# lxtGH/Video-K-Net

Hardware: AMD Instinct MI355X
Metric: frames/sec (S=3, N=100, 1024x2048) (higher is better)
Workload: dtype f32; 1 GPU; cfg2 video_knet_s3_r50: VideoKernelIterHead S=3, N=100 proposals + 17 stuff = 117 kernels, C=256, 1024x2048 frame -> 128x256 stride-8 features, ffn tracking link, x4 bilinear upsample of the final logits; streams_per_gpu=1, parallelism=frame-sharded dp1, x_storage=fp32

## Files before the change

include/vkn.h:

```cpp
#ifndef VKN_H
#define VKN_H
#include <stddef.h>
#include <stdint.h>

#ifdef __cplusplus
extern "C" {
#endif

#define VKN_VERSION 0x000600

#define VKN_OK 0
#define VKN_E_ARG (-1)
#define VKN_E_SHAPE (-2)
#define VKN_E_WORKSPACE (-3)
#define VKN_E_LAUNCH (-4)
#define VKN_E_ALIGN (-5)
#define VKN_E_RANGE (-6)

#define VKN_STATUS_RANGE 1u

#define VKN_FLAG_REF_KERNELS 1u
#define VKN_FLAG_EXACT_GEMM 2u
#define VKN_FLAG_LOGITS_HANDOFF 4u
#define VKN_FLAG_BITS_HANDOFF 16u
#define VKN_X_F32 0
#define VKN_X_F16 1
#define VKN_X_BF16 2
#define VKN_FLAG_X_F16 64u
#define VKN_FLAG_X_BF16 128u
#define VKN_FLAG_CHAIN_LAUNCHES 256u
#define VKN_FLAG_CHAIN_PERSISTENT 512u
#define VKN_FLAG_JOIN_EARLY 32768u
#define VKN_FLAG_SCALED_F16 16384u
#define VKN_FLAG_CHAIN_BF16X3 65536u
#define VKN_FLAG_CHAIN_KSPLIT 8192u
#define VKN_FLAG_SERIAL_LINK 32u
#define VKN_FLAG_CLIP_LINK 8u

#define VKN_FLAG_INIT_SEPARATE 131072u
#define VKN_FLAG_PHASE_A 1024u
#define VKN_FLAG_PHASE_B 2048u
#define VKN_FLAG_PHASE_C 4096u
#define VKN_FLAG_PHASE_MASK (VKN_FLAG_PHASE_A | VKN_FLAG_PHASE_B | VKN_FLAG_PHASE_C)

#define VKN_MAX_FCS 4

typedef struct VknDims {
// ... 366 lines not shown
```

video-k-net_amd/_lib.py:

```python
import ctypes
import os
import re
import subprocess

HERE = os.path.dirname(os.path.abspath(__file__))
CSRC = os.path.join(HERE, 'csrc')
LIBDIR = os.path.join(HERE, 'lib')
LIBPATH = os.path.join(LIBDIR, 'libvkn.so')
SOURCES = ('vkn_gather.hip', 'vkn_update.hip', 'vkn_decode.hip', 'vkn_fused.hip', 'vkn_init.hip', 'vkn_panoptic.hip', 'vkn_merge.hip', 'vkn_assign.hip', 'vkn_assign_lr.hip', 'vkn_tracker.hip', 'vkn_loss.hip', 'vkn_chain.hip', 'vkn_chain_h2.hip', 'vkn_ksplit.hip', 'vkn_train.hip', 'vkn_fpn.hip', 'vkn_optim.hip', 'vkn_tracktail.hip', 'vkn_trackloss.hip', 'vkn_gtprep.hip', 'vkn_api.hip')
HEADER = os.path.join(os.path.dirname(HERE), 'include', 'vkn.h')
TRACK_HEADER = os.path.join(os.path.dirname(HERE), 'include', 'vkn_track.h')
TRACK_TRAIN_HEADER = os.path.join(os.path.dirname(HERE), 'include', 'vkn_track_train.h')
GT_HEADER = os.path.join(os.path.dirname(HERE), 'include', 'vkn_gt.h')


class VknLibraryError(RuntimeError):
    pass


class VknError(RuntimeError):
    def __init__(self, code, msg):
        super().__init__(f'libvkn error {code}: {msg}')
        self.code = code


_SCALARS = {'int': ctypes.c_int, 'unsigned': ctypes.c_uint, 'unsigned int': ctypes.c_uint, 'size_t': ctypes.c_size_t,
            'float': ctypes.c_float, 'double': ctypes.c_double, 'long long': ctypes.c_longlong}
_POINTEES = {'void', 'char', 'unsigned char', 'int64_t'}
# ... 56 lines not shown
TRACK_PROTOS = {k: v for k, v in _protos.items() if k not in PROTOS}
TRACK_SYMBOLS = tuple(TRACK_PROTOS)
CONSTS.update({k: v for k, v in _consts.items() if k not in CONSTS})
with open(HEADER) as _f, open(TRACK_HEADER) as _g, open(TRACK_TRAIN_HEADER) as _h:
    _protos, _structs, _consts = read_header(_f.read() + '\n' + _g.read() + '\n' + _h.read())
TRACK_TRAIN_PROTOS = {k: v for k, v in _protos.items() if k not in PROTOS and k not in TRACK_PROTOS}
TRACK_TRAIN_SYMBOLS = tuple(TRACK_TRAIN_PROTOS)
TRACK_TRAIN_STRUCTS = {k: v for k, v in _structs.items() if k not in STRUCTS}
CONSTS.update({k: v for k, v in _consts.items() if k not in CONSTS})
with open(HEADER) as _f, open(TRACK_HEADER) as _g, open(TRACK_TRAIN_HEADER) as _h, open(GT_HEADER) as _i:
    _protos, _structs, _consts = read_header(_f.read() + '\n' + _g.read() + '\n' + _h.read() + '\n' + _i.read())
GT_PROTOS = {k: v for k, v in _protos.items() if k not in PROTOS and k not in TRACK_PROTOS and k not in TRACK_TRAIN_PROTOS}
GT_SYMBOLS = tuple(GT_PROTOS)
GT_STRUCTS = {k: v for k, v in _structs.items() if k not in STRUCTS and k not in TRACK_TRAIN_STRUCTS}
CONSTS.update({k: v for k, v in _consts.items() if k not in CONSTS})
GT_MAX_IMAGES = CONSTS['VKN_GT_MAX_IMAGES']
GT_MAX_CLASSES = CONSTS['VKN_GT_MAX_CLASSES']
GT_MAX_IDS = CONSTS['VKN_GT_MAX_IDS']
TRACK_LOSS_MAX_ROWS = CONSTS['VKN_TRACK_LOSS_MAX_ROWS']
TRACK_MAX_K = CONSTS['VKN_TRACK_MAX_K']
MAX_FCS = CONSTS['VKN_MAX_FCS']
SPLIT_MAX_ITEMS = CONSTS['VKN_SPLIT_MAX_ITEMS']
DW_MAX_ITEMS = CONSTS['VKN_DW_MAX_ITEMS']
ADAMW_GROUP_ROW = CONSTS['VKN_ADAMW_GROUP_ROW']
MIRRORS = {}
TRACK_TRAIN_MIRRORS = {}
GT_MIRRORS = {}


def _ctype(base, depth, where, result=False):
# ... 39 lines not shown

DEBUG_LIBPATH = os.path.join(LIBDIR, 'libvkn_debug.so')


def _hipcc(args, verbose=False, what='hipcc'):
    cmd = [os.environ.get('HIPCC', '/opt/rocm/bin/hipcc'), '--offload-arch=gfx950', *args]
    if verbose:
        print(' '.join(cmd), flush=True)
    r = subprocess.run(cmd, capture_output=True, text=True)
    if r.returncode != 0:
        raise VknLibraryError(f'{what} failed:\n' + r.stdout + r.stderr)


def _shared_deps(debug):
    exp = os.path.join(os.path.dirname(HERE), 'tools', 'experiments')
    return [HEADER, TRACK_HEADER, TRACK_TRAIN_HEADER, GT_HEADER] + ([os.path.join(exp, f) for f in os.listdir(exp)] if debug and os.path.isdir(exp) else [])


def _stale(path=None):
    path = path or LIBPATH
    if not os.path.exists(path):
        return True
    t = os.path.getmtime(path)
    deps = [os.path.join(CSRC, f) for f in os.listdir(CSRC)] + _shared_deps(path == DEBUG_LIBPATH)
    return any(os.path.getmtime(d) > t for d in deps if os.path.exists(d))


def _compile_objects(objdir, extra=(), force=False, verbose=False):
    from concurrent.futures import ThreadPoolExecutor
    os.makedirs(objdir, exist_ok=True)
    hdrs = [os.path.join(CSRC, f) for f in os.listdir(CSRC) if f.endswith('.h')] + _shared_deps('-DVKN_DEBUG' in extra)
# ... 38 lines not shown
    global _USE_DEBUG
    if _LIB is not None:
        raise VknLibraryError('use_debug() must be called before the library is first used')
    _USE_DEBUG = True


def lib():
    global _LIB
    if _LIB is not None:
        return _LIB
    path = DEBUG_LIBPATH if _USE_DEBUG else LIBPATH
    if not os.path.exists(path):
        raise VknLibraryError(f'{path} is missing — run `python -c "import __graft_entry__ as g; g.build()"` '
                              '(there is deliberately no CPU fallback)')
    L = ctypes.CDLL(path)
    for name, (result, params) in {**PROTOS, **TRACK_PROTOS, **TRACK_TRAIN_PROTOS, **GT_PROTOS}.items():
        fn = getattr(L, name)
        fn.restype = _ctype(*result, name, result=True)
        fn.argtypes = [POINTER_EXCEPTIONS.get((name, p)) or _ctype(base, depth, name) for p, base, depth in params]
    for name, mirror in {**MIRRORS, **TRACK_TRAIN_MIRRORS, **GT_MIRRORS}.items():
        probe = 'vkn_sizeof_' + re.sub(r'(?<!^)(?=[A-Z])', '_', name[3:]).lower()
        if probe not in PROTOS and probe not in TRACK_TRAIN_PROTOS and probe not in GT_PROTOS:
            raise VknLibraryError(f'include/vkn.h declares struct {name} without its size probe {probe}()')
        if getattr(L, probe)() != ctypes.sizeof(mirror):
            raise VknLibraryError(f'{path} does not match include/vkn.h: struct {name} is {getattr(L, probe)()} bytes in the library, '
                                  f'{ctypes.sizeof(mirror)} in the header')
    _LIB = L
    return L


def check(code):
# ... 3 lines not shown
```

video-k-net_amd/csrc/vkn_api.hip:

```cpp
#include "../../include/vkn.h"
#include "vkn_common.h"
#include "vkn_launch.h"

namespace {

struct Carver {
    char* base;
    size_t off;
    template <class T>
    T* take(size_t n) {
        off = (off + 255) & ~(size_t)255;
        T* p = base ? reinterpret_cast<T*>(base + off) : nullptr;
        off += n * sizeof(T);
        return p;
    }
};

inline bool aligned16(const void* p) { return (reinterpret_cast<uintptr_t>(p) & 15) == 0; }
inline int npt_of(int N) { return (N + 31) / 32 * 32; }

struct StageWs {
    float *part, *cntp, *xraw, *cnt, *xfeat, *params, *inputf, *ig, *ug, *f, *obj1, *qkv, *ao, *obj2, *h, *partial, *t1, *t2,
        *maskfeat, *kb, *kern32, *lq, *lkv, *lobj, *lupd, *lf;
    _Float16 *kfh, *kfl;
// ... 18 lines not shown
    const VknStageWeights* w = nullptr;
    const float *x = nullptr, *obj_in = nullptr;
    float *obj_out = nullptr, *cls_logits = nullptr, *x_feat_out = nullptr;
    bool cls_sigmoid = false;
    MasksFrom from = FROM_LOGITS;
    const float *masks_in = nullptr, *xfeat_in = nullptr;
    const unsigned* bits_in = nullptr;
    MasksTo to = TO_LOGITS;
    float* masks_out = nullptr;
    unsigned* bits_out = nullptr;
    float *kern_out = nullptr, *kb_out = nullptr;
    hipEvent_t prof0 = nullptr, prof1 = nullptr, obj_ready = nullptr;
    float* up_out = nullptr;
    int up_stride = 0, up_chunk = 0;
    bool* up_done = nullptr;
    const float* prev_obj = nullptr;
    float* track_out = nullptr;
    const VknStageWeights* link_pre = nullptr;
    const float* prev_pre = nullptr;
    const VknStageWeights* link_track = nullptr;
    int track_src = 0;
    bool keep_xfeat = false;
    const void* touch_next = nullptr;
    size_t touch_next_bytes = 0;
};

struct PrepW {
    const void *ft, *ftT, *dyn, *inp, *ig, *ug, *fc, *attn_in, *attn_out, *ffn1, *ffn2, *cls_fc[VKN_MAX_FCS], *fc_cls,
        *mask_fc[VKN_MAX_FCS], *fc_mask, *pa_in, *pa_in_kv, *pa_out, *lffn1, *lffn2;
    const void *dynft, *dec;
// ... 306 lines not shown
    const VknStageWeights* lw = link_track ? link_track : w;
    PrepW pw;
    VKN_TRY(carve_pw(d, lw, flags, &pw));
    return run_link(d, lw, pw, cur, prev, out, s, st, link_track ? (track_src == 2 ? cur : xfeat) : nullptr, flags);
}

int run_gather(const VknDims* d, const float* x, const float* masks, const unsigned* bits, const StageWs& s, unsigned flags,
               hipStream_t st, const void* touch = nullptr, size_t touch_bytes = 0) {
    const int B = d->B, N = d->N, C = d->C, P = d->H * d->W, xdt = xdt_of(flags);
    if (flags & VKN_FLAG_REF_KERNELS) return vkn_launch_gather_ref(x, masks, d->thr_logit, s.xraw, s.cnt, B, N, C, P, st);
    if (bits) return vkn_launch_gather_bits(x, bits, s.xraw, s.cnt, s.part, s.cntp, B, N, C, P, st, xdt, s.status, touch, touch_bytes);
    return vkn_launch_gather(x, masks, d->thr_logit, s.xraw, s.cnt, s.part, s.cntp, B, N, C, P, st, xdt, s.status, touch, touch_bytes);
}

int final_decode(const VknDims* d, const float* x, const StageWs& s, const float* kb, float* masks_out, unsigned flags,
                 hipStream_t st, hipEvent_t prof0, hipEvent_t prof1, float* up_out, int up_stride, int up_chunk, bool* up_done) {
    const int B = d->B, N = d->N, C = d->C, P = d->H * d->W;
    if ((flags & VKN_FLAG_REF_KERNELS) || (P & 1)) return vkn_launch_decode_ref(x, s.kern32, kb, masks_out, B, N, C, P, st);
    const int ch = (up_out && up_chunk > 0 && up_chunk < B) ? up_chunk : B;
    const size_t NPTC = (size_t)npt_of(N) * C;
    for (int b0 = 0; b0 < B; b0 += ch) {
        const int bn = (B - b0 < ch) ? B - b0 : ch;
        const float* xb = reinterpret_cast<const float*>(reinterpret_cast<const char*>(x) + (size_t)b0 * C * P * (xdt_of(flags) ? 2 : 4));
        if (b0 == 0 && prof0 && hipEventRecord(prof0, st) != hipSuccess) return VKN_E_LAUNCH;
        VKN_TRY(vkn_launch_decode(xb, s.kfh + b0 * NPTC, s.kfl + b0 * NPTC, kb ? kb + (size_t)b0 * N : nullptr,
                                  masks_out + (size_t)b0 * N * P, bn, N, C, P, st, xdt_of(flags)));
        if (b0 == 0 && prof1 && hipEventRecord(prof1, st) != hipSuccess) return VKN_E_LAUNCH;
        if (ch < B)
            VKN_TRY(vkn_launch_upsample(masks_out + (size_t)b0 * N * P,
                                        (flags & VKN_FLAG_SCALED_F16) ? reinterpret_cast<float*>(reinterpret_cast<_Float16*>(up_out) + (size_t)b0 * N * P * up_stride * up_stride)
                                                                      : up_out + (size_t)b0 * N * P * up_stride * up_stride,
                                        bn * N, d->H, d->W, up_stride, st, (flags & VKN_FLAG_SCALED_F16) ? 1 : 0));
    }
    if (ch < B && up_done) *up_done = true;
    return VKN_OK;
}

inline int persistent_min_row_tiles(const PrepW& pw, unsigned flags) {
    return (!(flags & VKN_FLAG_CHAIN_BF16X3) && pw.h2_scale && pw.h2[VKN_H2_DYNFT]) ? 22 : 64;
}
inline unsigned pw_off(const VknStageWeights* w, const void* p) {
    return (unsigned)(static_cast<const char*>(p) - static_cast<const char*>(w->prepared));
}
inline bool chain_weights_ok(const PrepW& pw, bool have_cls) {
    return pw.dynft && pw.dyn && pw.dec && pw.inp && pw.ig && pw.ug && pw.fc && pw.attn_in && pw.attn_out && pw.ffn1 && pw.ffn2 &&
           pw.cls_fc[0] && pw.mask_fc[0] && (!have_cls || pw.fc_cls);
}
inline bool chain_stage_ok(const VknDims* d, const VknStageWeights* w, const PrepW& pw, bool have_cls) {
    return chain_shape_ok(d) && w->prepared && w->prepared_bytes < (1ull << 31) && chain_weights_ok(pw, have_cls) && w->ffn1_w &&
           w->cls_ln_w[0] && w->mask_ln_w[0];
// ... 175 lines not shown
    pr[0] = ks_prob(s.t1, C, pw.lffn1, FF, 8, eps);
    pr[0].pro.ln_w[0] = w->pa_norm_w; pr[0].pro.ln_b[0] = w->pa_norm_b;
    pr[0].pro.side_out = s.lf; pr[0].pro.ld_side = C;
    pr[0].epi.bias = w->lffn1_b; pr[0].epi.act = 1; pr[0].epi.out = s.h; pr[0].epi.ldo = FF;
    VKN_TRY(vkn_launch_gemm_ks(pr, 1, 0, 0, 1, 0, M, st));
    const int kpw = (FF % 512 == 0) ? 2 : 1, zch = FF / (256 * kpw);
    pr[0] = ks_prob(s.h, FF, pw.lffn2, C, FF / 32, eps);
    pr[0].epi.out = s.partial; pr[0].epi.ldo = C;
    VKN_TRY(vkn_launch_gemm_ks(pr, 1, 0, zch, kpw, (long long)M * C, M, st));
    VknEpi e = mk_epi(d);
    e.bias = w->lffn2_b; e.resid = s.lf; e.ldr = C; e.ln_w = w->lffn_norm_w; e.ln_b = w->lffn_norm_b; e.out = out; e.ldo = C;
    return vkn_launch_rowepi(s.partial, zch, M, C, e, st);
}

int emit_masks(const VknDims* d, const StageCall& c, const StageWs& s, bool ref_decode, const float* kern32, const float* kb,
               const void* touch, size_t touch_bytes, unsigned flags, hipStream_t st) {
    const int B = d->B, N = d->N, C = d->C, P = d->H * d->W, xdt = xdt_of(flags);
    if (c.to == TO_KERNELS) {
        if (c.kb_out && kb && hipMemcpyAsync(c.kb_out, kb, (size_t)B * N * sizeof(float), hipMemcpyDeviceToDevice, st) != hipSuccess)
            return VKN_E_LAUNCH;
        return VKN_OK;
    }
    if (c.to == TO_NONE) return VKN_OK;
    if (ref_decode) return vkn_launch_decode_ref(c.x, kern32, kb, c.masks_out, B, N, C, P, st);
    if (c.to == TO_GATHER)
        return vkn_launch_fused_decode_gather(c.x, s.kfh, s.kfl, kb, d->thr_logit, s.xraw, s.cnt, s.part, s.cntp, B, N, C, P, st, xdt, s.status,
                                              touch, touch_bytes);
    if (c.to == TO_BITS) return vkn_launch_decode_bits(c.x, s.kfh, s.kfl, kb, c.bits_out, d->thr_logit, B, N, C, P, st, xdt);
    return final_decode(d, c.x, s, kb, c.masks_out, flags, st, c.prof0, c.prof1, c.up_out, c.up_stride, c.up_chunk, c.up_done);
}

int run_stage(const VknDims* d, const StageCall& c, const StageWs& s, unsigned flags, hipStream_t st) {
    const VknStageWeights* w = c.w;
    const int N = d->N, C = d->C, P = d->H * d->W, M = d->B * N;
    const bool ref = (flags & VKN_FLAG_REF_KERNELS) != 0;
    const bool chain_only = c.to == TO_KERNELS, given_xfeat = c.from == FROM_XFEAT;
    const bool ref_decode = ref || (P & 1) || chain_only;
    const bool has_ft = w->ft_w != nullptr;
    const bool have_cls = w->fc_cls_w && c.cls_logits;
    float* const cls_logits = have_cls ? c.cls_logits : nullptr;
    const bool pre_link = c.link_pre && c.prev_pre;
    const bool need_xfeat = (pre_link && c.link_pre->dyn_w) || (c.link_track && c.track_src == 1) || c.keep_xfeat;
    if (xdt_of(flags) && !chain_only && (ref || (P % 64) != 0)) return VKN_E_SHAPE;
    PrepW pw;
// ... 31 lines not shown
        obj_in = s.lobj;
    }

    const float* kb = has_ft ? s.kb : nullptr;
    float* const kern32 = ref_decode ? (chain_only ? c.kern_out : s.kern32) : nullptr;
    const bool link = c.prev_obj && c.track_out;
    if (fast) {
        const bool raw = !given_xfeat;
        if (fewrow) {
            VKN_TRY(run_chain_ks(d, w, pw, raw ? s.xraw : xfeat, raw, s.cnt, obj_in, c.obj_out, cls_logits, c.cls_sigmoid, kern32, s, st, c.obj_ready));
        } else {
            VKN_TRY(run_chain_fast(d, w, pw, raw ? s.xraw : xfeat, raw, s.cnt, obj_in, c.obj_out, cls_logits, c.cls_sigmoid, kern32, s, st,
                                   chain_h2(pw, flags, have_cls)));
            if (c.obj_ready && hipEventRecord(c.obj_ready, st) != hipSuccess) return VKN_E_LAUNCH;
        }
        VKN_TRY(emit_masks(d, c, s, ref_decode, s.kern32, kb, touch_nx, touch_nx_bytes, flags, st));
        if (link) VKN_TRY(run_track_link(d, s, st, c.obj_out, c.prev_obj, c.track_out, w, c.link_track, c.track_src, xfeat, flags));
        return VKN_OK;
    }

    VKN_TRY(run_updator(d, w, pw, xfeat, (comp && !given_xfeat) ? s.xraw : nullptr, s.cnt, obj_in, s.obj1, s, st));

    VKN_TRY(run_attention(d, s, s.obj1, s.obj1, d->heads, w->attn_in_w, pw.attn_in, nullptr, w->attn_in_b, w->attn_out_w,
                          pw.attn_out, w->attn_out_b, w->attn_norm_w, w->attn_norm_b, s.obj2, st));
    if (w->ffn1_w) {
        VKN_TRY(run_ffn(d, s, s.obj2, w->ffn1_w, pw.ffn1, w->ffn1_b, w->ffn2_w, pw.ffn2, w->ffn2_b, w->ffn_norm_w,
                        w->ffn_norm_b, c.obj_out, st));
    } else {
        if (hipMemcpyAsync(c.obj_out, s.obj2, (size_t)M * C * sizeof(float), hipMemcpyDeviceToDevice, st) != hipSuccess)
            return VKN_E_LAUNCH;
    }
// ... 205 lines not shown
                                   static_cast<hipStream_t>(stream));
}

int vkn_mask_decode_planes_f32(const float* x, const void* kf_hi, const void* kf_lo, const float* bias, float* out, int B,
                               int N, int C, int P, void* stream) {
    return vkn_mask_decode_planes_x(x, VKN_X_F32, kf_hi, kf_lo, bias, out, B, N, C, P, stream);
}

int vkn_mask_decode_planes_x(const void* x, int x_dtype, const void* kf_hi, const void* kf_lo, const float* bias, float* out, int B,
                             int N, int C, int P, void* stream) {
    if (!x || !kf_hi || !kf_lo || !out || B <= 0 || N <= 0 || C <= 0 || P <= 0 || x_dtype < 0 || x_dtype > 2) return VKN_E_ARG;
    if (!aligned16(x) || !aligned16(kf_hi) || !aligned16(kf_lo) || !aligned16(out)) return VKN_E_ALIGN;
    if (C % 32 != 0 || C > 256 || N > 256) return VKN_E_SHAPE;
    return vkn_launch_decode(static_cast<const float*>(x), static_cast<const _Float16*>(kf_hi), static_cast<const _Float16*>(kf_lo),
                             bias, out, B, N, C, P, static_cast<hipStream_t>(stream), x_dtype);
}

int vkn_decode_gather_supported(int C, int P) { return vkn_fused_supported(C, P); }

int vkn_decode_gather_f32(const float* x, const void* kf_hi, const void* kf_lo, const float* bias, float thr_logit,
                          float* xraw_out, float* cnt_out, int B, int N, int C, int P, void* ws, size_t ws_bytes, void* stream) {
    return vkn_decode_gather_x(x, VKN_X_F32, kf_hi, kf_lo, bias, thr_logit, xraw_out, cnt_out, B, N, C, P, ws, ws_bytes, stream);
}

int vkn_decode_gather_x(const void* xv, int x_dtype, const void* kf_hi, const void* kf_lo, const float* bias, float thr_logit,
                        float* xraw_out, float* cnt_out, int B, int N, int C, int P, void* ws, size_t ws_bytes, void* stream) {
    const float* x = static_cast<const float*>(xv);
    if (x_dtype < 0 || x_dtype > 2) return VKN_E_ARG;
    if (!x || !kf_hi || !kf_lo || !xraw_out || !cnt_out || B <= 0 || N <= 0 || C <= 0 || P <= 0) return VKN_E_ARG;
    if (!aligned16(x) || !aligned16(kf_hi) || !aligned16(kf_lo) || !aligned16(xraw_out)) return VKN_E_ALIGN;
// ... 499 lines not shown
    if (mask_preds_in == mask_preds_out || proposal_feats == obj_out) return VKN_E_ARG;
    StageWs s;
    float *mtmp, *otmp, *ctmp;
    unsigned* bits[2];
    const size_t need = carve_head(d, nullptr, &s, &mtmp, &otmp, &ctmp, bits);
    if (!ws || ws_bytes < need || !aligned16(ws)) return VKN_E_WORKSPACE;
    carve_head(d, static_cast<char*>(ws), &s, &mtmp, &otmp, &ctmp, bits);
    hipStream_t st = static_cast<hipStream_t>(stream);
    const bool use_bits = !(flags & (VKN_FLAG_REF_KERNELS | VKN_FLAG_LOGITS_HANDOFF)) && ((d->H * d->W) % 64) == 0;
    const bool use_fused = use_bits && !(flags & VKN_FLAG_BITS_HANDOFF) && vkn_fused_supported(d->C, d->H * d->W);

    const unsigned ph = flags & VKN_FLAG_PHASE_MASK;
    const bool do_a = !ph || (ph & VKN_FLAG_PHASE_A), do_b = !ph || (ph & VKN_FLAG_PHASE_B), do_c = !ph || (ph & VKN_FLAG_PHASE_C);
    if (ph && !(link_pre && (flags & VKN_FLAG_CLIP_LINK) && prev_obj)) return VKN_E_ARG;

    const float* m_in = mask_preds_in;
    const float* o_in = proposal_feats;
    SideStream* joined = nullptr;
    bool up_done = false;
    for (int sidx = 0; sidx < num_stages; ++sidx) {
        const bool last = (sidx == num_stages - 1);
        if (!last && !do_a) {
            const bool to_out_s = ((num_stages - 1 - sidx) & 1) == 0;
            m_in = to_out_s ? mask_preds_out : mtmp;
            o_in = to_out_s ? obj_out : otmp;
            continue;
        }
        const bool to_out = ((num_stages - 1 - sidx) & 1) == 0;
        float* m_out = to_out ? mask_preds_out : mtmp;
        float* o_out = to_out ? obj_out : otmp;
// ... 25 lines not shown
                } else {
                    c.touch_next = stages[sidx + 1].prepared;
                    c.touch_next_bytes = stages[sidx + 1].prepared_bytes;
                }
            }
        }
        hipEvent_t ev0 = last ? static_cast<hipEvent_t>(ev_decode_start) : nullptr;
        hipEvent_t ev1 = last ? static_cast<hipEvent_t>(ev_decode_stop) : nullptr;
        float* up_out = (last && scaled_out && upsample_stride > 1) ? scaled_out : nullptr;
        if (!seq) {
            c.to = (use_fused && !last) ? TO_GATHER : (b_out ? TO_BITS : TO_LOGITS);
            c.masks_out = m_out; c.bits_out = b_out;
            c.prof0 = ev0; c.prof1 = ev1; c.obj_ready = (prev && side) ? side->fork : nullptr;
            c.up_out = up_out; c.up_stride = upsample_stride; c.up_chunk = vkn_dbg_env("VKN_LAST_CHUNK", 0); c.up_done = &up_done;
            c.prev_obj = prev_in_stage; c.track_out = prev_in_stage ? track_out : nullptr;
            VKN_TRY(run_stage(d, c, s, flags, st));
        } else {
            const int N = d->N, C = d->C;
            if (do_a && c.from != FROM_GATHERED) VKN_TRY(run_gather(d, x, m_in, b_in, s, flags, st));
            VknDims d1 = *d;
            d1.B = 1;
            c.from = FROM_GATHERED;
            c.to = TO_NONE;
            c.keep_xfeat = ltrack && track_src == 1;
            c.link_track = nullptr;
            for (int b = 0; b < (do_b ? d->B : 0); ++b) {
                const size_t r = (size_t)b * N;
                const StageWs sb = frame_ws(s, d, b);
                c.obj_in = o_in + r * C; c.obj_out = o_out + r * C; c.cls_logits = cls_prob + r * d->ncls;
                c.prev_pre = b == 0 ? prev_obj : o_out + (r - N) * C;
                VKN_TRY(run_stage(&d1, c, sb, flags, st));
            }
            if (!do_c) return VKN_OK;
            if (prev && side && hipEventRecord(side->fork, st) != hipSuccess) return VKN_E_LAUNCH;
            VKN_TRY(final_decode(d, x, s, stages[sidx].ft_w ? s.kb : nullptr, m_out, flags, st, ev0, ev1, up_out, upsample_stride,
                                 vkn_dbg_env("VKN_LAST_CHUNK", 0), &up_done));
        }
        m_in = m_out;
        o_in = o_out;
        if (prev && link_after) {
            hipStream_t ls = side ? side->st : st;
            if (side && hipStreamWaitEvent(side->st, side->fork, 0) != hipSuccess) return VKN_E_LAUNCH;
            StageWs sl = s;
            if (side) {
                sl.lq = s.qkv;
                sl.lkv = s.qkv + (size_t)d->B * d->N * d->C;
                sl.t1 = s.obj1;
            }
            const float* pv = prev;
            if (clip) {
                const size_t fr = (size_t)d->N * d->C;
// ... 24 lines not shown
```

video-k-net_amd/csrc/vkn_decode.hip:

```cpp
#include "vkn_common.h"
#include "vkn_launch.h"

#define DEC_THREADS 512
#define DEC_WAVES 8
#define DEC_TILE 64
#define DEC_OPT_DEFAULT 1

typedef unsigned int u32x2 __attribute__((ext_vector_type(2)));
typedef unsigned int u32x4w __attribute__((ext_vector_type(4)));

template <int NB>
__device__ __forceinline__ void dec_emit_bits(const f32x16 (&acc)[2][NB], float thr, unsigned* __restrict__ wbase, int NPT,
                                              int lane) {
    constexpr int NH = (NB * 32 + 63) / 64;
    int w[2][NH];
#pragma unroll
    for (int t = 0; t < 2; ++t)
#pragma unroll
        for (int h = 0; h < NH; ++h) w[t][h] = 0;
#pragma unroll
    for (int nb = 0; nb < NB; ++nb)
#pragma unroll
        for (int r = 0; r < 16; ++r) {
            const unsigned long long m0 = __ballot(acc[0][nb][r] >= thr);
// ... 311 lines not shown
    for (int c = threadIdx.x; c < C; c += 256) {
        _Float16 h = (_Float16)0.f, l = (_Float16)0.f;
        if (n < N) vkn_split_f16(kern[((size_t)b * N + n) * C + c], h, l);
        kfh[(size_t)row * C + c] = h;
        kfl[(size_t)row * C + c] = l;
    }
}

int vkn_launch_decode(const float* x, const _Float16* kfh, const _Float16* kfl, const float* kb, float* out, int B,
                      int N, int C, int P, hipStream_t stream, int xdt) {
    return vkn_launch_decode_ex(x, kfh, kfl, kb, out, B, N, C, P, 0, N, stream, xdt);
}

static int decode_launch(const float* x, const _Float16* kfh, const _Float16* kfl, const float* kb, float* out, int B, int N,
                         int C, int P, int shared, int out_rows, unsigned* bits_out, float thr, hipStream_t stream, int xdt,
                         const float* oscale = nullptr);

int vkn_launch_decode_ex(const float* x, const _Float16* kfh, const _Float16* kfl, const float* kb, float* out, int B,
                         int N, int C, int P, int shared, int out_rows, hipStream_t stream, int xdt, const float* oscale) {
    return decode_launch(x, kfh, kfl, kb, out, B, N, C, P, shared, out_rows, nullptr, 0.f, stream, xdt, oscale);
}

int vkn_launch_decode_bits(const float* x, const _Float16* kfh, const _Float16* kfl, const float* kb, unsigned* bits_out,
                           float thr, int B, int N, int C, int P, hipStream_t stream, int xdt) {
    if (!bits_out || (P % 64) != 0) return VKN_E_SHAPE;
    return decode_launch(x, kfh, kfl, kb, nullptr, B, N, C, P, 0, N, bits_out, thr, stream, xdt);
}

static int decode_launch(const float* x, const _Float16* kfh, const _Float16* kfl, const float* kb, float* out, int B, int N,
                         int C, int P, int shared, int out_rows, unsigned* bits_out, float thr, hipStream_t stream, int xdt,
                         const float* oscale) {
    if (oscale && bits_out) return VKN_E_ARG;
    if (B <= 0 || N <= 0 || P <= 0 || out_rows < N) return VKN_E_ARG;
    if (xdt < 0 || xdt > 2) return VKN_E_ARG;
    if (C % 16 != 0 || C > 512 || P < 2 || (P & 1)) return VKN_E_SHAPE;
    if ((size_t)C * P * 4 >= ((size_t)1 << 31) || (size_t)N * P * 4 >= ((size_t)1 << 31)) return VKN_E_SHAPE;
    const int NPT = (N + 31) / 32 * 32;
    const VknDecodeStrides fs{shared ? 0 : (long long)NPT * C, shared ? 0 : (long long)N, (long long)out_rows * P};
    long long ppx = ((long long)B * P + 255) / 256;
    int px_per_wg = (int)((ppx + 511) / 512 * 512);
    if (px_per_wg < 512) px_per_wg = 512;
    const int ppw_dbg = vkn_dbg_env("VKN_DECODE_PXWG", 0);
    if (ppw_dbg >= 512) px_per_wg = ppw_dbg / 512 * 512;
    const int G2 = (P + px_per_wg - 1) / px_per_wg;
    const int xcd = vkn_dbg_env("VKN_DECODE_XCD", 1);
#ifdef VKN_DEBUG
    const bool wide = xdt == 0 && !bits_out && (P % D4_TILE) == 0 && (C % 64) == 0 && vkn_dbg_env("VKN_DECODE4", 0) != 0 &&
                      ((reinterpret_cast<uintptr_t>(x) | reinterpret_cast<uintptr_t>(out)) & 15) == 0;
#endif
    int znb = 0;
    if (!bits_out && NPT <= 128 && (long long)B * G2 <= 128) {
        znb = ((long long)B * G2 <= 64) ? 1 : 2;
        if (NPT % (znb * 32) != 0 || NPT / (znb * 32) < 2) znb = 0;
    }
    for (int n0 = 0; n0 < NPT; n0 += 128) {
        const int nb = znb ? znb : ((NPT - n0 >= 128) ? 4 : (NPT - n0) / 32);
        const size_t lds = (size_t)2 * nb * 32 * (C + 8) * sizeof(_Float16) + (size_t)nb * 32 * sizeof(float);
        dim3 grid(G2, B, znb ? NPT / (znb * 32) : 1);
#ifdef VKN_DEBUG
        if (wide) {
#define D4_CASE(NBV)                                                                                                       \
    case NBV: {                                                                                                            \
        VKN_ALLOW_FULL_LDS(k_decode4<NBV>);                                                                                \
        hipLaunchKernelGGL((k_decode4<NBV>), grid, dim3(D4_THREADS), lds, stream, x, kfh, kfl, kb, out, N, NPT, n0, C, P, \
                           px_per_wg, xcd, fs);                                                                            \
    } break;
            switch (nb) {
                D4_CASE(1)
// ... 139 lines not shown
```

video-k-net_amd/csrc/vkn_launch.h:

```cpp
#pragma once
#include <hip/hip_runtime.h>
#include <stddef.h>

struct VknEpi {
    const float* bias;
    const float* rowscale;
    const float* bias2;
    const float* resid;
    int ldr;
    const float* ln_w;
    const float* ln_b;
    int ln_from_col;
    float eps;
    int act;
    float* out;
    int ldo;
    const float* dot_vec;
    const float* dot_bias;
    float* dot_out;
    _Float16* plane_hi;
    _Float16* plane_lo;
    int rows_per_frame;
    int NPT;
};
// ... 30 lines not shown
                                   float* xraw, float* cnt, float* part, float* cntp, int B, int N, int C, int P,
                                   hipStream_t stream, int xdt = 0, int* status = nullptr, const void* touch = nullptr,
                                   size_t touch_bytes = 0);
int vkn_launch_gather(const float* x, const float* masks, float thr, float* xraw, float* cnt, float* part, float* cntp,
                      int B, int N, int C, int P, hipStream_t stream, int xdt = 0, int* status = nullptr, const void* touch = nullptr,
                      size_t touch_bytes = 0);
int vkn_launch_gather_ref(const float* x, const float* masks, float thr, float* xraw, float* cnt, int B, int N, int C,
                          int P, hipStream_t stream);
struct VknDecodeStrides {
    long long plane;
    long long kb;
    long long out;
};
int vkn_launch_decode_ex(const float* x, const _Float16* kfh, const _Float16* kfl, const float* kb, float* out, int B, int N,
                         int C, int P, int shared, int out_rows, hipStream_t stream, int xdt = 0, const float* oscale = nullptr);
int vkn_launch_decode_ref_ex(const float* x, const float* kern, const float* kb, float* out, int B, int N, int C, int P,
                             int shared, int out_rows, hipStream_t stream);
int vkn_launch_decode_bits(const float* x, const _Float16* kfh, const _Float16* kfl, const float* kb, unsigned* bits_out,
                           float thr, int B, int N, int C, int P, hipStream_t stream, int xdt = 0);
int vkn_launch_decode(const float* x, const _Float16* kfh, const _Float16* kfl, const float* kb, float* out, int B, int N,
                      int C, int P, hipStream_t stream, int xdt = 0);
int vkn_launch_decode_ref(const float* x, const float* kern, const float* kb, float* out, int B, int N, int C, int P,
                          hipStream_t stream);
int vkn_launch_split_planes(const float* kern, _Float16* kfh, _Float16* kfl, int B, int N, int C, hipStream_t stream);
int vkn_launch_gemm(const float* A, const float* A2, int lda, const float* W, const void* Wsplit, int M, int K, int Nout,
                    int ksplit, float* partial, const VknEpi& epi, hipStream_t stream);
int vkn_launch_gemm_group(const VknGemmProb* probs, int nprob, int M, int K, int ksplit, float* partial, hipStream_t stream);
size_t vkn_split_w3_bytes(int Nout, int K);
int vkn_launch_add2(const float* a, const float* b, float* out, size_t n, hipStream_t st);
int vkn_launch_add2_half(const void* a, const void* b, void* out, size_t n, int xdt, hipStream_t st);
// ... 128 lines not shown
```

video-k-net_amd/ops.py:

```python
import ctypes
import struct
import threading

import torch

from . import _lib
from ._lib import VknDims, VknStageWeights, check

_H = _lib.CONSTS
FLAG_REF_KERNELS = _H['VKN_FLAG_REF_KERNELS']
FLAG_EXACT_GEMM = _H['VKN_FLAG_EXACT_GEMM']
FLAG_LOGITS_HANDOFF = _H['VKN_FLAG_LOGITS_HANDOFF']
FLAG_BITS_HANDOFF = _H['VKN_FLAG_BITS_HANDOFF']
FLAG_CHAIN_LAUNCHES = _H['VKN_FLAG_CHAIN_LAUNCHES']
FLAG_CHAIN_PERSISTENT = _H['VKN_FLAG_CHAIN_PERSISTENT']
FLAG_JOIN_EARLY = _H['VKN_FLAG_JOIN_EARLY']
FLAG_SCALED_F16 = _H['VKN_FLAG_SCALED_F16']
FLAG_CHAIN_BF16X3 = _H['VKN_FLAG_CHAIN_BF16X3']
FLAG_INIT_SEPARATE = _H['VKN_FLAG_INIT_SEPARATE']
FLAG_CHAIN_KSPLIT = _H['VKN_FLAG_CHAIN_KSPLIT']
FLAG_SERIAL_LINK = _H['VKN_FLAG_SERIAL_LINK']

_tls = threading.local()


def _ptr(t):
    return ctypes.c_void_p(t.data_ptr()) if t is not None else ctypes.c_void_p(0)


def _stream():
    return ctypes.c_void_p(torch.cuda.current_stream().cuda_stream)
# ... 451 lines not shown
        check(_lib.lib().vkn_split_planes_f32(_ptr(k), _ptr(hi), _ptr(lo), B, N, C, _stream()))
    return hi, lo


def mask_decode_planes(x, hi, lo, N, bias=None, out=None):
    x, xdt = _req_x(x)
    B, C, H, W = x.shape
    if out is None:
        out = torch.empty((B, N, H, W), dtype=torch.float32, device=x.device)
    with torch.cuda.device(x.device):
        check(_lib.lib().vkn_mask_decode_planes_x(_ptr(x), xdt, _ptr(hi), _ptr(lo), _ptr(bias), _ptr(out), B, N, C, H * W,
                                                  _stream()))
    return out


def decode_gather(x, hi, lo, N, bias=None, hard_mask_thr=0.5):
    x, xdt = _req_x(x)
    B, C, H, W = x.shape
    P = H * W
    L = _lib.lib()
    xraw = torch.empty((B, N, C), dtype=torch.float32, device=x.device)
    cnt = torch.empty((B, N), dtype=torch.float32, device=x.device)
    ws = _workspace(L.vkn_gather_workspace_bytes(B, N, C, P), x.device, scratch=True)
    with torch.cuda.device(x.device):
        check(L.vkn_decode_gather_x(_ptr(x), xdt, _ptr(hi), _ptr(lo), _ptr(bias), thr_logit(hard_mask_thr), _ptr(xraw), _ptr(cnt),
                                    B, N, C, P, _ptr(ws), ws.numel(), _stream()))
    return xraw, cnt


def track_link(dims: VknDims, pack: StagePack, cur_obj, prev_obj, flags=0):
# ... 693 lines not shown
```

Measured before the change: 9725 frames/s.

## Cap final decode workgroups to reserve CUs for concurrent track link

Adds a workgroup-capped variant of the mask decode launch and uses it for the final-stage decode when a side-stream track link runs. By default, with a persistent chain, fp32 features and enough frames, it limits the decode grid so 64 CUs stay free for the link kernels on the side stream. The aim is to overlap linking with decoding instead of having the link wait for a full-device decode. The trade-off is fewer workgroups and larger per-workgroup pixel chunks for the decode, which may lengthen it.

```diff
diff --git a/include/vkn.h b/include/vkn.h
--- a/include/vkn.h
+++ b/include/vkn.h
@@ -31,6 +31,8 @@
 #define VKN_FLAG_CHAIN_LAUNCHES 256u
 #define VKN_FLAG_CHAIN_PERSISTENT 512u
 #define VKN_FLAG_JOIN_EARLY 32768u
+#define VKN_FLAG_LINK_RESERVE 262144u
+#define VKN_FLAG_LINK_NO_RESERVE 524288u
 #define VKN_FLAG_SCALED_F16 16384u
 #define VKN_FLAG_CHAIN_BF16X3 65536u
 #define VKN_FLAG_CHAIN_KSPLIT 8192u
diff --git a/include/vkn_decode.h b/include/vkn_decode.h
--- /dev/null
+++ b/include/vkn_decode.h
@@ -0,0 +1,18 @@
+#ifndef VKN_DECODE_H
+#define VKN_DECODE_H
+#include "vkn.h"
+
+#ifdef __cplusplus
+extern "C" {
+#endif
+
+int vkn_mask_decode_planes_wg_f32(const float* x, const void* kf_hi, const void* kf_lo, const float* bias, float* out, int B,
+                                  int N, int C, int P, int max_workgroups, void* stream);
+int vkn_mask_decode_planes_wg_x(const void* x, int x_dtype, const void* kf_hi, const void* kf_lo, const float* bias, float* out, int B,
+                                int N, int C, int P, int max_workgroups, void* stream);
+int vkn_decode_px_per_wg(int B, int P, int max_workgroups);
+
+#ifdef __cplusplus
+}
+#endif
+#endif
diff --git a/video-k-net_amd/_lib.py b/video-k-net_amd/_lib.py
--- a/video-k-net_amd/_lib.py
+++ b/video-k-net_amd/_lib.py
@@ -12,6 +12,7 @@
 TRACK_HEADER = os.path.join(os.path.dirname(HERE), 'include', 'vkn_track.h')
 TRACK_TRAIN_HEADER = os.path.join(os.path.dirname(HERE), 'include', 'vkn_track_train.h')
 GT_HEADER = os.path.join(os.path.dirname(HERE), 'include', 'vkn_gt.h')
+DECODE_HEADER = os.path.join(os.path.dirname(HERE), 'include', 'vkn_decode.h')
 
 
 class VknLibraryError(RuntimeError):
@@ -98,6 +99,9 @@
 GT_SYMBOLS = tuple(GT_PROTOS)
 GT_STRUCTS = {k: v for k, v in _structs.items() if k not in STRUCTS and k not in TRACK_TRAIN_STRUCTS}
 CONSTS.update({k: v for k, v in _consts.items() if k not in CONSTS})
+with open(DECODE_HEADER) as _f:
+    DECODE_PROTOS, _, _ = read_header(_f.read())
+DECODE_SYMBOLS = tuple(DECODE_PROTOS)
 GT_MAX_IMAGES = CONSTS['VKN_GT_MAX_IMAGES']
 GT_MAX_CLASSES = CONSTS['VKN_GT_MAX_CLASSES']
 GT_MAX_IDS = CONSTS['VKN_GT_MAX_IDS']
@@ -167,7 +171,7 @@
 
 def _shared_deps(debug):
     exp = os.path.join(os.path.dirname(HERE), 'tools', 'experiments')
-    return [HEADER, TRACK_HEADER, TRACK_TRAIN_HEADER, GT_HEADER] + ([os.path.join(exp, f) for f in os.listdir(exp)] if debug and os.path.isdir(exp) else [])
+    return [HEADER, TRACK_HEADER, TRACK_TRAIN_HEADER, GT_HEADER, DECODE_HEADER] + ([os.path.join(exp, f) for f in os.listdir(exp)] if debug and os.path.isdir(exp) else [])
 
 
 def _stale(path=None):
@@ -236,7 +240,7 @@
         raise VknLibraryError(f'{path} is missing — run `python -c "import __graft_entry__ as g; g.build()"` '
                               '(there is deliberately no CPU fallback)')
     L = ctypes.CDLL(path)
-    for name, (result, params) in {**PROTOS, **TRACK_PROTOS, **TRACK_TRAIN_PROTOS, **GT_PROTOS}.items():
+    for name, (result, params) in {**PROTOS, **TRACK_PROTOS, **TRACK_TRAIN_PROTOS, **GT_PROTOS, **DECODE_PROTOS}.items():
         fn = getattr(L, name)
         fn.restype = _ctype(*result, name, result=True)
         fn.argtypes = [POINTER_EXCEPTIONS.get((name, p)) or _ctype(base, depth, name) for p, base, depth in params]
diff --git a/video-k-net_amd/csrc/vkn_api.hip b/video-k-net_amd/csrc/vkn_api.hip
--- a/video-k-net_amd/csrc/vkn_api.hip
+++ b/video-k-net_amd/csrc/vkn_api.hip
@@ -1,4 +1,5 @@
 #include "../../include/vkn.h"
+#include "../../include/vkn_decode.h"
 #include "vkn_common.h"
 #include "vkn_launch.h"
 
@@ -56,6 +57,7 @@
     float* up_out = nullptr;
     int up_stride = 0, up_chunk = 0;
     bool* up_done = nullptr;
+    int link_reserve = 0;
     const float* prev_obj = nullptr;
     float* track_out = nullptr;
     const VknStageWeights* link_pre = nullptr;
@@ -392,7 +394,8 @@
 }
 
 int final_decode(const VknDims* d, const float* x, const StageWs& s, const float* kb, float* masks_out, unsigned flags,
-                 hipStream_t st, hipEvent_t prof0, hipEvent_t prof1, float* up_out, int up_stride, int up_chunk, bool* up_done) {
+                 hipStream_t st, hipEvent_t prof0, hipEvent_t prof1, float* up_out, int up_stride, int up_chunk, bool* up_done,
+                 int max_workgroups = 0) {
     const int B = d->B, N = d->N, C = d->C, P = d->H * d->W;
     if ((flags & VKN_FLAG_REF_KERNELS) || (P & 1)) return vkn_launch_decode_ref(x, s.kern32, kb, masks_out, B, N, C, P, st);
     const int ch = (up_out && up_chunk > 0 && up_chunk < B) ? up_chunk : B;
@@ -401,8 +404,8 @@
         const int bn = (B - b0 < ch) ? B - b0 : ch;
         const float* xb = reinterpret_cast<const float*>(reinterpret_cast<const char*>(x) + (size_t)b0 * C * P * (xdt_of(flags) ? 2 : 4));
         if (b0 == 0 && prof0 && hipEventRecord(prof0, st) != hipSuccess) return VKN_E_LAUNCH;
-        VKN_TRY(vkn_launch_decode(xb, s.kfh + b0 * NPTC, s.kfl + b0 * NPTC, kb ? kb + (size_t)b0 * N : nullptr,
-                                  masks_out + (size_t)b0 * N * P, bn, N, C, P, st, xdt_of(flags)));
+        VKN_TRY(vkn_launch_decode_wg(xb, s.kfh + b0 * NPTC, s.kfl + b0 * NPTC, kb ? kb + (size_t)b0 * N : nullptr,
+                                     masks_out + (size_t)b0 * N * P, bn, N, C, P, ch == B ? max_workgroups : 0, st, xdt_of(flags)));
         if (b0 == 0 && prof1 && hipEventRecord(prof1, st) != hipSuccess) return VKN_E_LAUNCH;
         if (ch < B)
             VKN_TRY(vkn_launch_upsample(masks_out + (size_t)b0 * N * P,
@@ -412,6 +415,20 @@
     }
     if (ch < B && up_done) *up_done = true;
     return VKN_OK;
+}
+
+#define VKN_LINK_RESERVE_CUS 64
+#define VKN_LINK_RESERVE_MIN_FRAMES 8
+inline int link_reserve_wg(const VknDims* d, int mode, bool persistent_chain, unsigned flags) {
+    const VknDecodeSplit dflt = vkn_decode_split(d->B, d->H * d->W, 0);
+    const long long grid = (long long)d->B * dflt.G2;
+    const int full = VKN_DECODE_CUS - VKN_LINK_RESERVE_CUS;
+    if (mode == 2) {
+        const long long q = grid * 3 / 4;
+        return (int)(q > full ? full : (q < d->B ? d->B : q));
+    }
+    if (mode != 1 || !persistent_chain || d->B < VKN_LINK_RESERVE_MIN_FRAMES || xdt_of(flags) != 0) return 0;
+    return grid == VKN_DECODE_CUS ? full : 0;
 }
 
 inline int persistent_min_row_tiles(const PrepW& pw, unsigned flags) {
@@ -617,7 +634,7 @@
 }
 
 int emit_masks(const VknDims* d, const StageCall& c, const StageWs& s, bool ref_decode, const float* kern32, const float* kb,
-               const void* touch, size_t touch_bytes, unsigned flags, hipStream_t st) {
+               const void* touch, size_t touch_bytes, unsigned flags, hipStream_t st, bool persistent_chain = false) {
     const int B = d->B, N = d->N, C = d->C, P = d->H * d->W, xdt = xdt_of(flags);
     if (c.to == TO_KERNELS) {
         if (c.kb_out && kb && hipMemcpyAsync(c.kb_out, kb, (size_t)B * N * sizeof(float), hipMemcpyDeviceToDevice, st) != hipSuccess)
@@ -630,7 +647,8 @@
         return vkn_launch_fused_decode_gather(c.x, s.kfh, s.kfl, kb, d->thr_logit, s.xraw, s.cnt, s.part, s.cntp, B, N, C, P, st, xdt, s.status,
                                               touch, touch_bytes);
     if (c.to == TO_BITS) return vkn_launch_decode_bits(c.x, s.kfh, s.kfl, kb, c.bits_out, d->thr_logit, B, N, C, P, st, xdt);
-    return final_decode(d, c.x, s, kb, c.masks_out, flags, st, c.prof0, c.prof1, c.up_out, c.up_stride, c.up_chunk, c.up_done);
+    return final_decode(d, c.x, s, kb, c.masks_out, flags, st, c.prof0, c.prof1, c.up_out, c.up_stride, c.up_chunk, c.up_done,
+                        link_reserve_wg(d, c.link_reserve, persistent_chain, flags));
 }
 
 int run_stage(const VknDims* d, const StageCall& c, const StageWs& s, unsigned flags, hipStream_t st) {
@@ -692,7 +710,7 @@
                                    chain_h2(pw, flags, have_cls)));
             if (c.obj_ready && hipEventRecord(c.obj_ready, st) != hipSuccess) return VKN_E_LAUNCH;
         }
-        VKN_TRY(emit_masks(d, c, s, ref_decode, s.kern32, kb, touch_nx, touch_nx_bytes, flags, st));
+        VKN_TRY(emit_masks(d, c, s, ref_decode, s.kern32, kb, touch_nx, touch_nx_bytes, flags, st, !fewrow));
         if (link) VKN_TRY(run_track_link(d, s, st, c.obj_out, c.prev_obj, c.track_out, w, c.link_track, c.track_src, xfeat, flags));
         return VKN_OK;
     }
@@ -928,6 +946,26 @@
     if (C % 32 != 0 || C > 256 || N > 256) return VKN_E_SHAPE;
     return vkn_launch_decode(static_cast<const float*>(x), static_cast<const _Float16*>(kf_hi), static_cast<const _Float16*>(kf_lo),
                              bias, out, B, N, C, P, static_cast<hipStream_t>(stream), x_dtype);
+}
+
+int vkn_mask_decode_planes_wg_f32(const float* x, const void* kf_hi, const void* kf_lo, const float* bias, float* out, int B,
+                                  int N, int C, int P, int max_workgroups, void* stream) {
+    return vkn_mask_decode_planes_wg_x(x, VKN_X_F32, kf_hi, kf_lo, bias, out, B, N, C, P, max_workgroups, stream);
+}
+
+int vkn_mask_decode_planes_wg_x(const void* x, int x_dtype, const void* kf_hi, const void* kf_lo, const float* bias, float* out, int B,
+                                int N, int C, int P, int max_workgroups, void* stream) {
+    if (!x || !kf_hi || !kf_lo || !out || B <= 0 || N <= 0 || C <= 0 || P <= 0 || x_dtype < 0 || x_dtype > 2 || max_workgroups < 0)
+        return VKN_E_ARG;
+    if (!aligned16(x) || !aligned16(kf_hi) || !aligned16(kf_lo) || !aligned16(out)) return VKN_E_ALIGN;
+    if (C % 32 != 0 || C > 256 || N > 256) return VKN_E_SHAPE;
+    return vkn_launch_decode_wg(static_cast<const float*>(x), static_cast<const _Float16*>(kf_hi), static_cast<const _Float16*>(kf_lo),
+                                bias, out, B, N, C, P, max_workgroups, static_cast<hipStream_t>(stream), x_dtype);
+}
+
+int vkn_decode_px_per_wg(int B, int P, int max_workgroups) {
+    if (B <= 0 || P <= 0 || max_workgroups < 0) return VKN_E_ARG;
+    return vkn_decode_split(B, P, max_workgroups).px_per_wg;
 }
 
 int vkn_decode_gather_supported(int C, int P) { return vkn_fused_supported(C, P); }
@@ -1457,6 +1495,7 @@
     const bool do_a = !ph || (ph & VKN_FLAG_PHASE_A), do_b = !ph || (ph & VKN_FLAG_PHASE_B), do_c = !ph || (ph & VKN_FLAG_PHASE_C);
     if (ph && !(link_pre && (flags & VKN_FLAG_CLIP_LINK) && prev_obj)) return VKN_E_ARG;
 
+    const int link_reserve = (flags & VKN_FLAG_LINK_NO_RESERVE) ? 0 : ((flags & VKN_FLAG_LINK_RESERVE) ? 2 : 1);
     const float* m_in = mask_preds_in;
     const float* o_in = proposal_feats;
     SideStream* joined = nullptr;
@@ -1512,6 +1551,7 @@
             c.prof0 = ev0; c.prof1 = ev1; c.obj_ready = (prev && side) ? side->fork : nullptr;
             c.up_out = up_out; c.up_stride = upsample_stride; c.up_chunk = vkn_dbg_env("VKN_LAST_CHUNK", 0); c.up_done = &up_done;
             c.prev_obj = prev_in_stage; c.track_out = prev_in_stage ? track_out : nullptr;
+            c.link_reserve = (prev && side) ? link_reserve : 0;
             VKN_TRY(run_stage(d, c, s, flags, st));
         } else {
             const int N = d->N, C = d->C;
@@ -1532,7 +1572,7 @@
             if (!do_c) return VKN_OK;
             if (prev && side && hipEventRecord(side->fork, st) != hipSuccess) return VKN_E_LAUNCH;
             VKN_TRY(final_decode(d, x, s, stages[sidx].ft_w ? s.kb : nullptr, m_out, flags, st, ev0, ev1, up_out, upsample_stride,
-                                 vkn_dbg_env("VKN_LAST_CHUNK", 0), &up_done));
+                                 vkn_dbg_env("VKN_LAST_CHUNK", 0), &up_done, link_reserve_wg(d, (prev && side) ? link_reserve : 0, false, flags)));
         }
         m_in = m_out;
         o_in = o_out;
diff --git a/video-k-net_amd/csrc/vkn_decode.hip b/video-k-net_amd/csrc/vkn_decode.hip
--- a/video-k-net_amd/csrc/vkn_decode.hip
+++ b/video-k-net_amd/csrc/vkn_decode.hip
@@ -349,7 +349,7 @@
 
 static int decode_launch(const float* x, const _Float16* kfh, const _Float16* kfl, const float* kb, float* out, int B, int N,
                          int C, int P, int shared, int out_rows, unsigned* bits_out, float thr, hipStream_t stream, int xdt,
-                         const float* oscale = nullptr);
+                         const float* oscale = nullptr, int max_workgroups = 0);
 
 int vkn_launch_decode_ex(const float* x, const _Float16* kfh, const _Float16* kfl, const float* kb, float* out, int B,
                          int N, int C, int P, int shared, int out_rows, hipStream_t stream, int xdt, const float* oscale) {
@@ -362,19 +362,38 @@
     return decode_launch(x, kfh, kfl, kb, nullptr, B, N, C, P, 0, N, bits_out, thr, stream, xdt);
 }
 
+VknDecodeSplit vkn_decode_split(int B, int P, int max_workgroups) {
+    const long long ppx = ((long long)B * P + VKN_DECODE_CUS - 1) / VKN_DECODE_CUS;
+    int px_per_wg = (int)((ppx + 511) / 512 * 512);
+    if (px_per_wg < 512) px_per_wg = 512;
+    int G2 = (P + px_per_wg - 1) / px_per_wg;
+    if (max_workgroups > 0 && (long long)B * G2 > max_workgroups) {
+        const int G = max_workgroups / B > 0 ? max_workgroups / B : 1;
+        const int share = (P + G - 1) / G;
+        px_per_wg = (share + 511) / 512 * 512;
+        G2 = (P + px_per_wg - 1) / px_per_wg;
+    }
+    return VknDecodeSplit{px_per_wg, G2};
+}
+
+int vkn_launch_decode_wg(const float* x, const _Float16* kfh, const _Float16* kfl, const float* kb, float* out, int B, int N,
+                         int C, int P, int max_workgroups, hipStream_t stream, int xdt) {
+    return decode_launch(x, kfh, kfl, kb, out, B, N, C, P, 0, N, nullptr, 0.f, stream, xdt, nullptr, max_workgroups);
+}
+
 static int decode_launch(const float* x, const _Float16* kfh, const _Float16* kfl, const float* kb, float* out, int B, int N,
                          int C, int P, int shared, int out_rows, unsigned* bits_out, float thr, hipStream_t stream, int xdt,
-                         const float* oscale) {
+                         const float* oscale, int max_workgroups) {
     if (oscale && bits_out) return VKN_E_ARG;
+    if (max_workgroups < 0) return VKN_E_ARG;
     if (B <= 0 || N <= 0 || P <= 0 || out_rows < N) return VKN_E_ARG;
     if (xdt < 0 || xdt > 2) return VKN_E_ARG;
     if (C % 16 != 0 || C > 512 || P < 2 || (P & 1)) return VKN_E_SHAPE;
     if ((size_t)C * P * 4 >= ((size_t)1 << 31) || (size_t)N * P * 4 >= ((size_t)1 << 31)) return VKN_E_SHAPE;
     const int NPT = (N + 31) / 32 * 32;
     const VknDecodeStrides fs{shared ? 0 : (long long)NPT * C, shared ? 0 : (long long)N, (long long)out_rows * P};
-    long long ppx = ((long long)B * P + 255) / 256;
-    int px_per_wg = (int)((ppx + 511) / 512 * 512);
-    if (px_per_wg < 512) px_per_wg = 512;
+    const VknDecodeSplit split = vkn_decode_split(B, P, max_workgroups);
+    int px_per_wg = split.px_per_wg;
     const int ppw_dbg = vkn_dbg_env("VKN_DECODE_PXWG", 0);
     if (ppw_dbg >= 512) px_per_wg = ppw_dbg / 512 * 512;
     const int G2 = (P + px_per_wg - 1) / px_per_wg;
@@ -387,6 +406,7 @@
     if (!bits_out && NPT <= 128 && (long long)B * G2 <= 128) {
         znb = ((long long)B * G2 <= 64) ? 1 : 2;
         if (NPT % (znb * 32) != 0 || NPT / (znb * 32) < 2) znb = 0;
+        if (znb && max_workgroups > 0 && (long long)B * G2 * (NPT / (znb * 32)) > max_workgroups) znb = 0;
     }
     for (int n0 = 0; n0 < NPT; n0 += 128) {
         const int nb = znb ? znb : ((NPT - n0 >= 128) ? 4 : (NPT - n0) / 32);
diff --git a/video-k-net_amd/csrc/vkn_launch.h b/video-k-net_amd/csrc/vkn_launch.h
--- a/video-k-net_amd/csrc/vkn_launch.h
+++ b/video-k-net_amd/csrc/vkn_launch.h
@@ -68,6 +68,13 @@
 };
 int vkn_launch_decode_ex(const float* x, const _Float16* kfh, const _Float16* kfl, const float* kb, float* out, int B, int N,
                          int C, int P, int shared, int out_rows, hipStream_t stream, int xdt = 0, const float* oscale = nullptr);
+#define VKN_DECODE_CUS 256
+struct VknDecodeSplit {
+    int px_per_wg, G2;
+};
+VknDecodeSplit vkn_decode_split(int B, int P, int max_workgroups);
+int vkn_launch_decode_wg(const float* x, const _Float16* kfh, const _Float16* kfl, const float* kb, float* out, int B, int N,
+                         int C, int P, int max_workgroups, hipStream_t stream, int xdt = 0);
 int vkn_launch_decode_ref_ex(const float* x, const float* kern, const float* kb, float* out, int B, int N, int C, int P,
                              int shared, int out_rows, hipStream_t stream);
 int vkn_launch_decode_bits(const float* x, const _Float16* kfh, const _Float16* kfl, const float* kb, unsigned* bits_out,
diff --git a/video-k-net_amd/ops.py b/video-k-net_amd/ops.py
--- a/video-k-net_amd/ops.py
+++ b/video-k-net_amd/ops.py
@@ -15,6 +15,8 @@
 FLAG_CHAIN_LAUNCHES = _H['VKN_FLAG_CHAIN_LAUNCHES']
 FLAG_CHAIN_PERSISTENT = _H['VKN_FLAG_CHAIN_PERSISTENT']
 FLAG_JOIN_EARLY = _H['VKN_FLAG_JOIN_EARLY']
+FLAG_LINK_RESERVE = _H['VKN_FLAG_LINK_RESERVE']
+FLAG_LINK_NO_RESERVE = _H['VKN_FLAG_LINK_NO_RESERVE']
 FLAG_SCALED_F16 = _H['VKN_FLAG_SCALED_F16']
 FLAG_CHAIN_BF16X3 = _H['VKN_FLAG_CHAIN_BF16X3']
 FLAG_INIT_SEPARATE = _H['VKN_FLAG_INIT_SEPARATE']
@@ -496,6 +498,24 @@
     return out
 
 
+def mask_decode_planes_wg(x, hi, lo, N, max_workgroups, bias=None, out=None):
+    x, xdt = _req_x(x)
+    B, C, H, W = x.shape
+    if out is None:
+        out = torch.empty((B, N, H, W), dtype=torch.float32, device=x.device)
+    with torch.cuda.device(x.device):
+        check(_lib.lib().vkn_mask_decode_planes_wg_x(_ptr(x), xdt, _ptr(hi), _ptr(lo), _ptr(bias), _ptr(out), B, N, C, H * W,
+                                                     int(max_workgroups), _stream()))
+    return out
+
+
+def decode_px_per_wg(B, P, max_workgroups=0):
+    r = _lib.lib().vkn_decode_px_per_wg(int(B), int(P), int(max_workgroups))
+    if r < 0:
+        check(r)
+    return r
+
+
 def decode_gather(x, hi, lo, N, bias=None, hard_mask_thr=0.5):
     x, xdt = _req_x(x)
     B, C, H, W = x.shape
```

After: 10010 frames/s (median of 6 runs). +2.9%, better.
